# syguan96/DynaBOA

Measured on AMD Instinct MI355X. Metric: adapted frames/sec, whole job (3 inner + 1 outer step, bs=1 per sequence, first-order; synthetic 224x224 stream, no 3DPW assets in the image: PA-MPJPE on 3DPW not measured), higher is better.
Workload: dtype f32

## Files before the change

dynaboa_amd/csrc/adapt_step.hip:

```cpp
#include <math.h>
#include <stdlib.h>
#include <string.h>

#include <algorithm>
#include <chrono>
#include <string>
#include <vector>

#include "dyb_common.h"
#include "dyb_stepper_options.h"

extern "C" {
size_t dyb_hmr_param_floats(const void*);
size_t dyb_hmr_act_floats(const void*);
size_t dyb_hmr_workspace_bytes(const void*);
int dyb_hmr_forward_train(void*, const float*, const float*, const float*, int, float*, void*, size_t, unsigned long long, unsigned long long, float,
                          hipStream_t);
long long dyb_hmr_act_offset_rotmat(const void*);
long long dyb_hmr_act_offset_state(const void*);
size_t dyb_lbs_saved_floats(int);
size_t dyb_lbs_bwd_workspace_bytes(int);
int dyb_lbs_fwd(const float* const*, const int* const*, const float*, int, const float*, float*, float*, float*, int, hipStream_t);
int dyb_lbs_bwd(const float* const*, const int* const*, const float*, const float*, const float*, const float*, float*, float*, int,
                int, void*, size_t, hipStream_t);
// ... 222 lines not shown
  int teacher_train = 0;
  unsigned long long drop_seed = 0, drop_off = 0;
  long long drop_used = 0;
  double drop_p = 0.5;
  volatile float* gate_host = nullptr;
  float* gate_log = nullptr;
  float* feat5_out = nullptr;
  int (*retrieve)(void*, int, const void**) = nullptr;
  int (*retrieve_rep)(void*, int, int, const void**) = nullptr;
  void* retrieve_user = nullptr;
  const float *bank_img = nullptr, *bank_kp = nullptr, *bank_pose = nullptr, *bank_betas = nullptr, *bank_pose3d = nullptr;
  const float *bank_centers = nullptr, *bank_inv_norm = nullptr;
  const int *bank_member_ptr = nullptr, *bank_member_idx = nullptr;
  int* bank_picks = nullptr;
  int bank_items = 0, bank_clusters = 0, bank_members = 0, bank_pick_capacity = 0, bank_on_device = 1;
  unsigned long long bank_seed = 0;
  unsigned long long bank_draw[DYB_MAX_REPLICAS] = {};
  char* retr_ws = nullptr;
  FeatCosArgs fca{};
  float gate_seq = 0.f;
  Pass lvl0{}, ex{}, hist{}, teach{};
  float *grads2 = nullptr, *grads3 = nullptr, *zeros = nullptr, *ex_rot = nullptr;
  const float *lvl_g2 = nullptr, *lvl_g3 = nullptr;
  float *ext_rot = nullptr, *ext_shape = nullptr, *ext_cam = nullptr, *ext_joints = nullptr;
  float *exg_rot = nullptr, *exg_shape = nullptr, *exg_cam = nullptr, *exg_joints = nullptr;
  float *hg_cam = nullptr, *hg_joints = nullptr;
  float *vals_t = nullptr, *vals_m = nullptr, *vals_l = nullptr;
  int nrep = 1;
  int active[DYB_MAX_REPLICAS] = {};
  int nactive = 0;
  long long adam_t_rep[DYB_MAX_REPLICAS] = {};
  size_t blob = 0;
  float* in_stage[12] = {};
  double lr = 3e-6, beta1 = 0.5, beta2 = 0.9, eps = 1e-8, fastlr = 8e-6, w2d = 10.0, wshape = 2e-6, wpose = 1e-4;
  long long adam_t = 0;
  float *theta = nullptr, *adam_m = nullptr, *adam_v = nullptr;
  const float* init_state = nullptr;
  const float* smpl_f[3][7] = {};
  const int* smpl_i[3][3] = {};
  const float *gmm_means = nullptr, *gmm_prec = nullptr, *gmm_logw = nullptr, *j_h36m = nullptr;
  const int* j14 = nullptr;
  float *records = nullptr, *loss_log = nullptr;
  const char* logs_base = nullptr;
  size_t logs_bytes = 0;
  int record_capacity = 0, loss_capacity = 0;
  float* results = nullptr;
  int result_capacity = 0;
  char* wsp = nullptr;
  bool bound = false;
  Pass main{}, fin{};
  float *theta_fast = nullptr, *grads = nullptr;
  float* theta_fast2 = nullptr;
  int fuse_fast = 1;
  std::vector<DybSpan> fused_spans, upd_spans;
  int fuse_adam = 1;
  int fuse_ema = 1;
  float* adam_sc = nullptr;
  bool adam_prepared = false;
  float pre_ss[DYB_MAX_REPLICAS], pre_bc[DYB_MAX_REPLICAS];
  float *gt_rot = nullptr, *gt_verts[3] = {}, *gt_joints = nullptr, *gt_saved = nullptr, *gt17[2] = {};
  DybEvents* ev = nullptr;
  hipEvent_t e_theta = nullptr, e_side = nullptr, e_gt = nullptr;
  int upd_overlap = 1;
  int par_passes = 1, par_max_replicas = DYB_MAX_REPLICAS;
  hipStream_t par_stream[2] = {nullptr, nullptr};
  hipEvent_t par_ev[9] = {nullptr, nullptr, nullptr, nullptr, nullptr, nullptr, nullptr, nullptr, nullptr};
  bool out_in_main = false;
  int share_dyn_fwd = 1;
  hipEvent_t e_upd = nullptr;
  DybFwdGates gates{};
  bool gates_pending = false;
  int wgrad_defer = 1;
  bool defer_pending = false;
  int n_deferred = 0;
  int upd_late = 1;
  struct Upd {
    bool adam = false, ema = false;
    const float *g2 = nullptr, *g3 = nullptr;
    const float* p = nullptr;
    float* out = nullptr;
    float ss[DYB_MAX_REPLICAS] = {}, bc[DYB_MAX_REPLICAS] = {};
  };
  struct LateUpd {
    Upd u;
    hipStream_t aux = nullptr;
    DybRep scope{};
  } late;
  size_t grp_bounds[2] = {0, 0};
  bool side_pending = false;
  struct Tail {
    bool on = false;
    const float* image = nullptr;
    const long long* gender = nullptr;
    int slot = 0;
    bool metrics = false;
    int loss_slot = -1;
  } tail;
  struct GtJob {
    bool on = false;
    const float *pose = nullptr, *betas = nullptr;
  } gtjob;
  hipStream_t tail_stream = nullptr;
  std::string err;
  double h_fwd = 0, h_bwd = 0, h_head = 0, h_update = 0, h_tail = 0, h_total = 0;
  long long h_frames = 0;
};
struct HostTimer {
  double& acc;
  std::chrono::steady_clock::time_point t0;
  explicit HostTimer(double& a) : acc(a), t0(std::chrono::steady_clock::now()) {}
  ~HostTimer() { acc += std::chrono::duration<double, std::milli>(std::chrono::steady_clock::now() - t0).count(); }
};

static size_t a64(size_t v) { return (v + 63) & ~(size_t)63; }
#define BANK_MAX_CHUNKS 256
static bool bank_bound(const Stepper& S) { return S.bank_img && S.bank_on_device; }
static const char* opt_env(const char* name) { return name ? getenv(name) : nullptr; }

static size_t carve(Stepper& S, char* base) {
  size_t off = 0;
  auto take_f = [&](size_t nfloats) -> float* {
    float* p = base ? reinterpret_cast<float*>(base + off) : nullptr;
    off += a64(nfloats) * sizeof(float);
    return p;
  };
  auto take_b = [&](size_t nbytes) -> char* {
    char* p = base ? base + off : nullptr;
    off += a64((nbytes + 3) / 4) * sizeof(float);
    return p;
  };
  const size_t B = (size_t)S.B;
  auto pass = [&](Pass& P, bool with_grad) {
    P.acts = take_f(S.act_floats);
// ... 20 lines not shown
  pass(S.main, true);
  pass(S.fin, false);
  S.theta_fast = take_f(S.n_params);
  S.theta_fast2 = S.fuse_fast ? take_f(S.n_params) : nullptr;
  S.adam_sc = take_f(64);
  S.grads = take_f(S.n_params);
  S.gt_rot = take_f(B * 24 * 9);
  for (int i = 0; i < 3; ++i) S.gt_verts[i] = take_f(B * NV * 3);
  S.gt_joints = take_f(B * NJ * 3);
  S.gt_saved = take_f(S.lbs_saved);
  S.gt17[0] = take_f(B * 51);
  S.gt17[1] = take_f(B * 51);
  if (S.full) {
    S.lvl0 = S.main;
    S.lvl0.acts = take_f(S.act_floats);
    pass(S.ex, true);
    pass(S.hist, true);
    pass(S.teach, false);
    S.grads2 = take_f(S.n_params);
    S.grads3 = take_f(S.n_params);
    S.zeros = take_f(B * 216);
    S.ex_rot = take_f(B * 216);
    S.ext_rot = take_f(B * 216); S.ext_shape = take_f(B * 10); S.ext_cam = take_f(B * 3); S.ext_joints = take_f(B * NJ * 3);
    S.exg_rot = take_f(B * 216); S.exg_shape = take_f(B * 10); S.exg_cam = take_f(B * 3); S.exg_joints = take_f(B * NJ * 3);
    S.hg_cam = take_f(B * 3); S.hg_joints = take_f(B * NJ * 3);
    S.vals_t = take_f(8); S.vals_m = take_f(8); S.vals_l = take_f(8);
  }
  if (S.nrep > 1) {
    S.in_stage[0] = take_f(B * 3 * (size_t)S.H * S.W);
    S.in_stage[1] = take_f(B * NJ * 3);
    S.in_stage[2] = take_f(B * 72);
    S.in_stage[3] = take_f(B * 10);
    S.in_stage[4] = take_f(B * 2);
    if (S.full) {
      S.in_stage[5] = take_f(B * 3 * (size_t)S.H * S.W);
      S.in_stage[6] = take_f(B * NJ * 3);
      S.in_stage[7] = take_f(B * 3 * (size_t)S.H * S.W);
      S.in_stage[8] = take_f(B * NJ * 3);
      S.in_stage[9] = take_f(B * 72);
      S.in_stage[10] = take_f(B * 10);
      S.in_stage[11] = take_f(B * 24 * 4);
    }
  } else if (S.full && S.bank_img) {
    S.in_stage[7] = take_f(B * 3 * (size_t)S.H * S.W);
    S.in_stage[8] = take_f(B * NJ * 3);
    S.in_stage[9] = take_f(B * 72);
    S.in_stage[10] = take_f(B * 10);
    S.in_stage[11] = take_f(B * 24 * 4);
  }
  S.retr_ws = (S.full && S.bank_img) ? take_b(dyb_retrieve_workspace_bytes(S.nrep, BANK_MAX_CHUNKS, 1)) : nullptr;
  return off;
}

extern "C" int dyb_stepper_create(void* plan, int B, int H, int W, void** out) {
  DYB_REQUIRE(plan && out && B > 0 && B <= 64, DYB_ERR_ARG);
  Stepper* S = new Stepper();
  S->plan = plan; S->B = B; S->H = H; S->W = W;
  S->n_params = dyb_hmr_param_floats(plan);
  S->act_floats = dyb_hmr_act_floats(plan);
  S->ws_bytes = dyb_hmr_workspace_bytes(plan);
  S->off_rot = (size_t)dyb_hmr_act_offset_rotmat(plan);
  S->off_state = (size_t)dyb_hmr_act_offset_state(plan);
  S->lbs_saved = dyb_lbs_saved_floats(B);
  S->lbs_wsb = dyb_lbs_bwd_workspace_bytes(B);
  S->ev = dyb_hmr_events_create(plan);
  dyb_hmr_param_groups(plan, S->grp_bounds);
#define DYB_OPT_ENV_(member, name, env, type, locked, doc) \
  if (const char* e = opt_env(env)) S->member = atoi(e);
  DYB_STEPPER_OPTIONS_I(DYB_OPT_ENV_)
#undef DYB_OPT_ENV_
  if (!S->ev || hipEventCreateWithFlags(&S->e_theta, hipEventDisableTiming) != hipSuccess ||
      hipEventCreateWithFlags(&S->e_side, hipEventDisableTiming) != hipSuccess ||
      hipEventCreateWithFlags(&S->e_gt, hipEventDisableTiming) != hipSuccess ||
      hipEventCreateWithFlags(&S->e_upd, hipEventDisableTiming) != hipSuccess ||
      hipEventCreateWithFlags(&S->gates.ev[0], hipEventDisableTiming) != hipSuccess ||
      hipEventCreateWithFlags(&S->gates.ev[1], hipEventDisableTiming) != hipSuccess ||
      hipEventCreateWithFlags(&S->gates.mid, hipEventDisableTiming) != hipSuccess ||
      hipEventCreateWithFlags(&S->ev->l4, hipEventDisableTiming) != hipSuccess ||
      hipEventCreateWithFlags(&S->ev->reg, hipEventDisableTiming) != hipSuccess) {
    delete S;
    return DYB_ERR_LAUNCH;
  }
  *out = S;
  return DYB_OK;
}
extern "C" void dyb_stepper_destroy(void* stepper) {
  Stepper* S = reinterpret_cast<Stepper*>(stepper);
  if (!S) return;
  dyb_hmr_events_destroy(S->ev);
  if (S->e_theta) (void)hipEventDestroy(S->e_theta);
  if (S->e_side) (void)hipEventDestroy(S->e_side);
  if (S->e_gt) (void)hipEventDestroy(S->e_gt);
  if (S->e_upd) (void)hipEventDestroy(S->e_upd);
  if (S->gates.ev[0]) (void)hipEventDestroy(S->gates.ev[0]);
  if (S->gates.ev[1]) (void)hipEventDestroy(S->gates.ev[1]);
  if (S->gates.mid) (void)hipEventDestroy(S->gates.mid);
  for (int i = 0; i < 9; ++i) if (S->par_ev[i]) (void)hipEventDestroy(S->par_ev[i]);
  for (int i = 0; i < 2; ++i) if (S->par_stream[i]) (void)hipStreamDestroy(S->par_stream[i]);
  delete S;
}

extern "C" int dyb_stepper_set_i(void* stepper, const char* key, long long v) {
  Stepper* S = reinterpret_cast<Stepper*>(stepper);
  DYB_REQUIRE(S && key, DYB_ERR_ARG);
  const std::string k(key);
#define DYB_OPT_SET_I_(member, name, env, type, locked, doc) \
  if (k == name) {                                           \
    DYB_REQUIRE(!(locked) || !S->bound, DYB_ERR_ARG);        \
    S->member = (int)v;                                      \
    return DYB_OK;                                           \
  }
  DYB_STEPPER_OPTIONS_I(DYB_OPT_SET_I_)
#undef DYB_OPT_SET_I_
  if (k == "adam_step") {
    S->adam_t = v;
    for (int r = 0; r < DYB_MAX_REPLICAS; ++r) S->adam_t_rep[r] = v;
  }
  else if (k.compare(0, 10, "adam_step_") == 0) {
    const int r = atoi(k.c_str() + 10);
    DYB_REQUIRE(r >= 0 && r < DYB_MAX_REPLICAS, DYB_ERR_ARG);
    S->adam_t_rep[r] = v;
    S->adam_t = 0;
    for (int q = 0; q < S->nrep || q <= r; ++q)
      if (S->adam_t_rep[q] > S->adam_t) S->adam_t = S->adam_t_rep[q];
  }
// ... 195 lines not shown
  for (int g = 0; g < 3; ++g)
    RUN(dyb_lbs_fwd(S.smpl_f[g], S.smpl_i[g], gt_betas, 10, S.gt_rot, S.gt_verts[g], S.gt_joints, S.gt_saved, S.B, st));
  RUN(dyb_regress_joints(S.j_h36m, S.gt_verts[1], S.gt17[0], 17, S.B, st));
  return dyb_regress_joints(S.j_h36m, S.gt_verts[2], S.gt17[1], 17, S.B, st);
}
static int record_metrics(Stepper& S, Pass& P, const long long* gender, int slot, hipStream_t st) {
  DYB_REQUIRE(slot >= 0 && slot < S.record_capacity, DYB_ERR_ARG);
  RUN(dyb_regress_joints(S.j_h36m, P.verts, P.pred17, 17, S.B, st));
  float* rec = S.records + (size_t)slot * a64((size_t)S.B * 85 + 1);
  const DybRep& Rp = dyb_rep_current();
  hipLaunchKernelGGL(metric_record_kernel, dim3(1, 1, Rp.n), dim3(256), 0, st, P.pred17, S.gt17[0], S.gt17[1], gender, S.j14, P.verts,
                     S.gt_verts[0], rec, S.B, Rp);
  DYB_CHECK_LAUNCH();
  return DYB_OK;
}

static int pack_result(Stepper& S, Pass& P, int loss_slot, hipStream_t st) {
  if (!S.results || loss_slot < 0) return DYB_OK;
  float* row = S.results + (size_t)(loss_slot % S.result_capacity) * S.B * RESULT_FLOATS;
  return dyb_result_pack(P.acts + S.off_rot, P.acts + S.off_state, P.verts, row, S.B, st);
}

static int issue_side_work(Stepper& S, hipStream_t side) {
  if (S.tail.on) {
    HIPOK(hipStreamWaitEvent(side, S.e_theta, 0));
    RUN(pass_forward(S, S.fin, S.theta, S.tail.image, side, false));
    if (S.tail.metrics) RUN(record_metrics(S, S.fin, S.tail.gender, S.tail.slot, side));
    RUN(pack_result(S, S.fin, S.tail.loss_slot, side));
    HIPOK(hipEventRecord(S.e_side, side));
    S.side_pending = true;
    S.tail.on = false;
  }
  if (S.gtjob.on) {
    RUN(gt_meshes(S, S.gtjob.pose, S.gtjob.betas, side));
    HIPOK(hipEventRecord(S.e_gt, side));
    S.gtjob.on = false;
  }
  return DYB_OK;
}
static bool spans_touch(const Stepper& S, size_t lo, size_t hi) {
  for (const DybSpan& sp : S.upd_spans)
    if (sp.off < hi && sp.off + sp.n > lo) return true;
  return false;
}
template <class Emit>
static int walk_gaps(const Stepper& S, size_t lo, size_t hi, Emit emit) {
  DYB_REQUIRE(lo % 4 == 0 && hi % 4 == 0, DYB_ERR_UNSUPPORTED);
  DybFwSegs t{};
  auto flush = [&]() -> int {
    if (t.n == 0) return DYB_OK;
    const int rc = emit(t);
    t.n = 0;
    return rc;
  };
  auto add = [&](size_t a, size_t b) -> int {
    if (a >= b) return DYB_OK;
    DYB_REQUIRE(a % 4 == 0 && b % 4 == 0 && (b - a) / 4 < 0xffffffffull && a / 4 < 0xffffffffull, DYB_ERR_UNSUPPORTED);
    if (t.n == DYB_FW_MAX_SEGS) RUN(flush());
    t.start4[t.n] = (unsigned)(a / 4); t.count4[t.n] = (unsigned)((b - a) / 4); ++t.n;
    return DYB_OK;
  };
  size_t at = lo;
  for (const DybSpan& sp : S.upd_spans) {
    if (sp.off + sp.n <= at) continue;
    if (sp.off >= hi) break;
    DYB_REQUIRE(sp.off >= lo && sp.off + sp.n <= hi, DYB_ERR_UNSUPPORTED);
// ... 300 lines not shown
        const void* one[5] = {nullptr, nullptr, nullptr, nullptr, nullptr};
        if (S.retrieve_rep(S.retrieve_user, level_index, r, one) != 0) return DYB_ERR_ARG;
        for (int k = 0; k < 5; ++k) {
          DYB_REQUIRE(one[k], DYB_ERR_ARG);
          exin[k * DYB_MAX_REPLICAS + r] = one[k];
        }
      }
      RUN(stage_inputs(S, exin, DYB_MAX_REPLICAS, IN_EX_IMG, 5, st));
      for (int k = 0; k < 5; ++k) C.in[IN_EX_IMG + k] = S.in_stage[IN_EX_IMG + k];
    } else if (S.retrieve) {
      DYB_REQUIRE(S.feat5_out && S.nrep == 1, DYB_ERR_ARG);
      RUN(dyb_scale_add(nullptr, P.acts + S.fca.off[5], nullptr, S.feat5_out, (size_t)0 + (size_t)B * 2048, st));
      const void* exin[5] = {nullptr, nullptr, nullptr, nullptr, nullptr};
      if (S.retrieve(S.retrieve_user, level_index, exin) != 0) return DYB_ERR_ARG;
      for (int k = 0; k < 5; ++k) C.in[IN_EX_IMG + k] = exin[k];
    }
    DYB_REQUIRE(C.in[IN_EX_IMG] && C.in[IN_EX_KP] && C.in[IN_EX_POSE] && C.in[IN_EX_BETAS] && C.in[IN_EX_POSE3D], DYB_ERR_ARG);
    RUN(label_pass_forward_and_term(st, true));
  }
  if (C.losslog && S.full) {
    if (par && label) HIPOK(hipStreamWaitEvent(st, S.par_ev[4], 0));
    hipLaunchKernelGGL(level_log_kernel, dim3(1, 1, dyb_rep_current().n), dim3(64), 0, st, (const float*)P.losses,
                       teacher ? (const float*)S.vals_t : nullptr, motion ? (const float*)S.vals_m : nullptr,
                       label ? (const float*)S.vals_l : nullptr, (float)S.teacher_w, (float)S.motion_w, (float)S.label_w,
                       C.losslog + 16 * level_index, dyb_rep_current());
    DYB_CHECK_LAUNCH();
  }
  {
    HostTimer t(S.h_bwd);
    S.fused_spans.clear();
    DybWgradUpdate upd{};
    if (fused_epilogues(S) && !upper && S.fuse_fast && S.theta_fast2) {
      upd = DybWgradUpdate{S.grads, S.n_params * sizeof(float), cur, nxt, (float)S.fastlr, &S.fused_spans};
    } else if (fused_epilogues(S) && upper && S.fuse_adam && cur != S.theta && !C.side && S.nrep > 1) {
      RUN(adam_prepare(S, st));
      upd = DybWgradUpdate{S.grads, S.n_params * sizeof(float), S.theta, S.theta, 0.f, &S.fused_spans};
      upd.adam_m = S.adam_m; upd.adam_v = S.adam_v; upd.adam_sc = S.adam_sc;
      upd.b1 = (float)S.beta1; upd.b2 = (float)S.beta2; upd.eps = (float)S.eps;
    }
    DybWgradUpdateScope fuse(upd);
    RUN(pass_backward_ext(S, P, cur, S.grads, true, ext ? S.ext_rot : nullptr, ext ? S.ext_shape : nullptr, ext ? S.ext_cam : nullptr,
                          ext ? S.ext_joints : nullptr, st, aux));
  }
  S.lvl_g2 = S.lvl_g3 = nullptr;
  if (motion) {
    if (par) HIPOK(hipStreamWaitEvent(st, S.par_ev[3], 0));
    else RUN(pass_backward_ext(S, S.hist, cur, S.grads2, false, nullptr, nullptr, S.hg_cam, S.hg_joints, st, aux));
    S.lvl_g2 = S.grads2;
  }
  if (label) {
    if (par) HIPOK(hipStreamWaitEvent(st, S.par_ev[5], 0));
    else RUN(pass_backward_ext(S, S.ex, cur, S.grads3, false, S.exg_rot, S.exg_shape, S.exg_cam, S.exg_joints, st, aux));
    if (S.lvl_g2) S.lvl_g3 = S.grads3;
    else S.lvl_g2 = S.grads3;
  }
  tails.armed = false;
  return DYB_OK;
}
static int outer_update(Stepper& S, hipStream_t st, hipStream_t aux) {
  return weight_update(S, true, nullptr, nullptr, st, aux, S.full && S.use_teacher && S.teacher);
}
static int gate_cosine(Stepper& S, const float* actsA, const float* actsB, float* log_row, float* cos12, hipStream_t st) {
  DYB_REQUIRE(S.gate_host, DYB_ERR_ARG);
  const DybRep& R = dyb_rep_current();
  S.gate_seq += 1.f;
  hipLaunchKernelGGL(feat_cos_kernel, dim3(15, 1, R.n), dim3(1024), 0, st, actsA, actsB, S.fca, 1e-12f, log_row, S.gate_host, S.gate_seq, R);
  DYB_CHECK_LAUNCH();
// ... 54 lines not shown
    arena(S.loss_log, (size_t)S.loss_capacity * (S.full ? 16 : 4) * rows * sizeof(float));
    if (S.full) {
      arena(S.gate_log, (size_t)S.loss_capacity * (1 + S.optim_steps) * 16 * sizeof(float));
      arena(S.feat5_out, (size_t)S.B * 2048 * sizeof(float));
    }
  }
  DYB_REQUIRE(!overflow, DYB_ERR_UNSUPPORTED);
  *out = R;
  return DYB_OK;
}
extern "C" int dyb_stepper_set_active(void* stepper, const int* idx, int n) {
  Stepper* S = reinterpret_cast<Stepper*>(stepper);
  DYB_REQUIRE(S && n >= 0 && n <= S->nrep && (n == 0 || idx), DYB_ERR_ARG);
  for (int i = 0; i < n; ++i) DYB_REQUIRE(idx[i] >= 0 && idx[i] < S->nrep && (i == 0 || idx[i] > idx[i - 1]), DYB_ERR_ARG);
  S->nactive = n;
  for (int i = 0; i < n; ++i) S->active[i] = idx[i];
  return DYB_OK;
}
static int active_set(const Stepper& S, int* idx) {
  if (S.nactive > 0) {
    for (int i = 0; i < S.nactive; ++i) idx[i] = S.active[i];
    return S.nactive;
  }
  for (int i = 0; i < S.nrep; ++i) idx[i] = i;
  return S.nrep;
}

static int frame_step(Stepper& S, LevelCtx& C, int record_slot, int loss_slot, int* extra, hipStream_t st, hipStream_t aux, hipStream_t side) {
  const bool metrics = S.metrics != 0;
  DYB_REQUIRE(C.in[IN_IMAGE] && C.in[IN_KP], DYB_ERR_ARG);
  DYB_REQUIRE(!metrics || (C.in[IN_GT_POSE] && C.in[IN_GT_BETAS] && C.in[IN_GENDER]), DYB_ERR_ARG);
  S.out_in_main = false;
  if (!S.use_side || side == st) side = nullptr;
  const float* image = (const float*)C.in[IN_IMAGE];
  const long long* gender = (const long long*)C.in[IN_GENDER];
  const int K = S.inner_step;
  const int rows = K + 1 + (S.full && S.dynamic ? S.optim_steps : 0);
  C.losslog = (S.loss_log && loss_slot >= 0 && loss_slot < S.loss_capacity) ? S.loss_log + (size_t)loss_slot * (S.full ? 16 : 4) * rows : nullptr;
  C.side = side;
  int slot = record_slot;
  const DybRep outer = dyb_rep_current();
  for (int i = 0; i < outer.n; ++i) extra[dyb_rep_phys(outer, i)] = 0;
  if (metrics) {
    if (side) {
      S.gtjob.on = true; S.gtjob.pose = (const float*)C.in[IN_GT_POSE]; S.gtjob.betas = (const float*)C.in[IN_GT_BETAS];
    } else {
      RUN(gt_meshes(S, (const float*)C.in[IN_GT_POSE], (const float*)C.in[IN_GT_BETAS], st));
    }
  }
  C.gt_waited = !(metrics && side);
  HostTimer t_all(S.h_total);
  ++S.h_frames;
  const float* cur = S.theta;
  for (int i = 0; i <= K; ++i) {
    Pass& P = (i == 0 && S.full && S.dynamic) ? S.lvl0 : S.main;
    float* nxt = (fused_epilogues(S) && S.fuse_fast && S.theta_fast2 && cur == S.theta_fast) ? S.theta_fast2 : S.theta_fast;
    RUN(level(S, C, P, cur, nxt, i == K, i, (metrics && S.eval_lower && i > 0) ? slot++ : -1, st, aux));
    if (i == 0 && side) {
      HostTimer t(S.h_tail);
      RUN(issue_side_work(S, side));
    }
    if (i < K) {
      HostTimer t(S.h_update);
      RUN(weight_update(S, false, cur, nxt, st, aux));
      cur = nxt;
    }
  }
  {
    HostTimer t_tail(S.h_tail);
    if (S.side_pending) {
      HIPOK(hipStreamWaitEvent(st, S.e_side, 0));
      S.side_pending = false;
    }
    RUN(outer_update(S, st, side ? nullptr : aux));
    if (side) {
      HIPOK(hipEventRecord(S.e_theta, st));
      S.tail.on = true; S.tail.image = image; S.tail.gender = gender; S.tail.slot = slot++; S.tail.metrics = metrics;
      S.tail.loss_slot = loss_slot;
      S.tail_stream = side;
      return DYB_OK;
    }
    RUN(pass_forward(S, S.fin, S.theta, image, st));
    RUN(settle_update(S, st));
    if (metrics) RUN(record_metrics(S, S.fin, gender, slot++, st));
    RUN(pack_result(S, S.fin, loss_slot, st));
  }
  if (!(S.full && S.dynamic)) return DYB_OK;
  float* glog = (S.gate_log && loss_slot >= 0 && loss_slot < S.loss_capacity) ? S.gate_log + (size_t)loss_slot * (1 + S.optim_steps) * 16 : nullptr;
  DYB_REQUIRE(glog, DYB_ERR_ARG);
  float cos12[DYB_MAX_REPLICAS];
  RUN(gate_cosine(S, S.lvl0.acts, S.fin.acts, glog, cos12, st));
  int cont[DYB_MAX_REPLICAS], ncont = 0;
  for (int i = 0; i < outer.n; ++i)
    if (1.f - cos12[dyb_rep_phys(outer, i)] > (float)S.cos_thr) cont[ncont++] = dyb_rep_phys(outer, i);
  int step = 0;
  Pass* post = &S.fin;
  while (ncont > 0) {
    ++step;
    if (step > S.optim_steps) {
      for (int i = 0; i < ncont; ++i) extra[cont[i]] = S.optim_steps + 1;
      break;
    }
    {
      DybRep sub = outer;
      dyb_rep_set_map(sub, cont, ncont);
      DybRepScope scope(sub);
      Pass up = S.main;
// ... 10 lines not shown
      RUN(pack_result(S, *nxt, loss_slot, st));
      post = nxt;
      S.out_in_main = (post == &S.main);
    }
    ++slot;
    int m = 0;
    for (int i = 0; i < ncont; ++i) {
      extra[cont[i]] = step;
      if (1.f - cos12[cont[i]] > (float)S.cos_thr) cont[m++] = cont[i];
    }
    ncont = m;
  }
  return DYB_OK;
}
static int adapt(Stepper& S, const void* const* inputs, int nk, int record_slot, int loss_slot, int* extra_steps, hipStream_t st,
                 hipStream_t aux, hipStream_t side) {
  RUN(check_ready(S));
  DYB_REQUIRE((nk == IN_COUNT) == (S.full != 0) && (!S.full || S.B <= 16), DYB_ERR_UNSUPPORTED);
  struct DrawGuard {
    Stepper& S;
    unsigned long long saved[DYB_MAX_REPLICAS];
    bool ok = false;
    explicit DrawGuard(Stepper& s) : S(s) { memcpy(saved, S.bank_draw, sizeof saved); }
    ~DrawGuard() { if (!ok) memcpy(S.bank_draw, saved, sizeof saved); }
  } draws(S);
  const int n = S.nrep;
  int extra[DYB_MAX_REPLICAS] = {};
  LevelCtx C{};
  int rc;
  if (n == 1) {
    for (int k = 0; k < nk; ++k) C.in[k] = inputs[k];
    rc = frame_step(S, C, record_slot, loss_slot, extra, st, aux, side);
  } else {
    DYB_REQUIRE(!(S.use_side && side && side != st), DYB_ERR_UNSUPPORTED);
    int act[DYB_MAX_REPLICAS];
    const int na = active_set(S, act);
    auto have = [&](int r, int k0, int k1) {
      for (int k = k0; k <= k1; ++k)
        if (k >= nk || !inputs[k * n + r]) return false;
      return true;
    };
    const bool have_gt = have(act[0], IN_GT_POSE, IN_GENDER), have_hist = have(act[0], IN_HIST_IMAGE, IN_HIST_KP),
               have_ex = have(act[0], IN_EX_IMG, IN_EX_POSE3D);
    for (int i = 0; i < na; ++i) {
      DYB_REQUIRE(have(act[i], IN_IMAGE, IN_KP), DYB_ERR_ARG);
      DYB_REQUIRE(have(act[i], IN_GT_POSE, IN_GENDER) == have_gt && have(act[i], IN_HIST_IMAGE, IN_HIST_KP) == have_hist &&
                  have(act[i], IN_EX_IMG, IN_EX_POSE3D) == have_ex, DYB_ERR_UNSUPPORTED);
    }
    DybRep R{};
    RUN(make_scope(S, act, na, &R));
    DybRepScope scope(R);
    RUN(stage_inputs(S, inputs, n, IN_IMAGE, 5, st));
    if (have_hist) RUN(stage_inputs(S, inputs + (size_t)IN_HIST_IMAGE * n, n, IN_HIST_IMAGE, 2, st));
    if (have_ex) RUN(stage_inputs(S, inputs + (size_t)IN_EX_IMG * n, n, IN_EX_IMG, 5, st));
    for (int k = 0; k < nk; ++k) {
      const bool on = k <= IN_KP || (k <= IN_GENDER ? have_gt : k <= IN_HIST_KP ? have_hist : have_ex);
      C.in[k] = on ? S.in_stage[k] : nullptr;
    }
    rc = frame_step(S, C, record_slot, loss_slot, extra, st, aux, side);
  }
  if (extra_steps)
    for (int r = 0; r < n; ++r) extra_steps[r] = extra[r];
  draws.ok = rc == DYB_OK;
  return rc;
}
extern "C" int dyb_stepper_adapt_frame(void* stepper, const float* image, const float* kp2d, const float* gt_pose,
                                       const float* gt_betas, const long long* gender, int record_slot, int loss_slot,
                                       hipStream_t st, hipStream_t aux, hipStream_t side) {
  Stepper* S = reinterpret_cast<Stepper*>(stepper);
  DYB_REQUIRE(S && image && kp2d && S->nrep == 1, DYB_ERR_ARG);
  const void* inputs[5] = {image, kp2d, gt_pose, gt_betas, gender};
  return adapt(*S, inputs, 5, record_slot, loss_slot, nullptr, st, aux, side);
}
extern "C" int dyb_stepper_adapt_frames(void* stepper, const void* const* inputs, int record_slot, int loss_slot, hipStream_t st,
                                        hipStream_t aux, hipStream_t side) {
  Stepper* S = reinterpret_cast<Stepper*>(stepper);
  DYB_REQUIRE(S && inputs, DYB_ERR_ARG);
  return adapt(*S, inputs, 5, record_slot, loss_slot, nullptr, st, aux, side);
}
extern "C" int dyb_stepper_adapt_frame_full(void* stepper, const void* const* inputs, int record_slot, int loss_slot, int* extra_steps,
                                            hipStream_t st, hipStream_t aux) {
  Stepper* S = reinterpret_cast<Stepper*>(stepper);
  DYB_REQUIRE(S && inputs && extra_steps, DYB_ERR_ARG);
  DYB_REQUIRE(S->nrep == 1, DYB_ERR_UNSUPPORTED);
  return adapt(*S, inputs, IN_COUNT, record_slot, loss_slot, extra_steps, st, aux, nullptr);
// ... 31 lines not shown
```

dynaboa_amd/csrc/dyb_stepper_options.h:

```cpp
#pragma once
#define DYB_STEPPER_OPTIONS_I(X)                                                                                                              \
  X(n_iter, "n_iter", nullptr, I, 0, "iterations of the HMR regressor (1 .. 3)")                                                              \
  X(inner_step, "inner_step", nullptr, I, 0, "lower levels per frame (0 .. 16)")                                                              \
  X(eval_lower, "eval_lower", nullptr, I, 0, "a metric record after every inner step")                                                        \
  X(use_side, "use_side", nullptr, I, 0, "one sequence, frame-loss set: final inference and ground-truth meshes on the side stream")          \
  X(metrics, "metrics", nullptr, I, 0, "metric records at all")                                                                               \
  X(upd_overlap, "upd_overlap", "DYB_UPD_OVERLAP", I, 0, "replica groups: weight updates by arena ranges beside the next forward")            \
  X(upd_late, "upd_late", "DYB_UPD_LATE", I, 0, "the last range (layer4 + regressor) is issued when the consuming forward reaches layer3")    \
  X(wgrad_defer, "wgrad_defer", "DYB_WGRAD_DEFER", I, 0, "layer4 / regressor weight gradients behind the backward's join, beside the next forward") \
  X(fuse_fast, "fuse_fast", "DYB_FUSE_FAST", I, 1, "frame-loss set: lower levels' weight gradients write the fast weights themselves (second fast buffer)") \
  X(fuse_adam, "fuse_adam", "DYB_FUSE_ADAM", I, 0, "frame-loss set, replica groups: the outer level's weight gradients apply Adam in place")  \
  X(fuse_ema, "fuse_ema", "DYB_FUSE_EMA", I, 0, "the teacher's EMA inside the Adam pass")                                                     \
  X(par_passes, "par_passes", "DYB_PAR_PASSES", I, 0, "full set: history and exemplar passes on two streams of the stepper's own")            \
  X(par_max_replicas, "par_max_replicas", "DYB_PAR_MAX_REPLICAS", I, 0, "largest launch set that still runs the parallel passes")             \
  X(share_dyn_fwd, "share_dyn_fwd", "DYB_SHARE_DYN_FWD", I, 0, "dynamic loop: a step's upper level reuses the previous final inference as its forward") \
  X(full, "full", nullptr, I, 1, "the reference's full term set (teacher / motion / labelled exemplars / dynamic loop): sizes the workspace")  \
  X(temporal_lower, "temporal_lower", nullptr, I, 0, "teacher / motion terms on the lower levels")                                            \
  X(temporal_upper, "temporal_upper", nullptr, I, 0, "teacher / motion terms on the upper level")                                             \
  X(use_teacher, "use_teacher", nullptr, I, 0, "mean-teacher term and the teacher's EMA")                                                     \
  X(teacher_train, "teacher_train", nullptr, I, 0, "teacher forwards with live dropout (keys: drop_seed, drop_offset)")                       \
  X(use_motion, "use_motion", nullptr, I, 0, "motion term against the frame `interval` steps back")                                           \
  X(interval, "interval", nullptr, I, 0, "distance of the history frame (bookkeeping of the caller)")                                         \
  X(mix_lower, "mix_lower", nullptr, I, 0, "labelled-exemplar term on the lower levels")                                                      \
  X(mix_upper, "mix_upper", nullptr, I, 0, "labelled-exemplar term on the upper level")                                                       \
  X(dynamic, "dynamic", nullptr, I, 0, "dynamic loop: repeat the upper level while feature 12 still moves")                                   \
  X(optim_steps, "optim_steps", nullptr, I, 0, "its iteration limit")                                                                         \
  X(kp_set, "kp_set", nullptr, I, 0, "keypoint window of the 2D term and the motion term: 0 gt24 (joints 25..48) | 1 op25 (joints 0..24)")   \
  X(record_capacity, "record_capacity", nullptr, I, 0, "metric-record slots behind `records`")                                                \
  X(loss_capacity, "loss_capacity", nullptr, I, 0, "frames behind `loss_log` / `gate_log`")                                                   \
  X(result_capacity, "result_capacity", nullptr, I, 0, "rows behind `results` (a frame's final inferences go to row loss_slot mod this)")      \
  X(bank_items, "bank_items", nullptr, I, 0, "exemplar bank: items in the five tables")                                                       \
  X(bank_clusters, "bank_clusters", nullptr, I, 0, "exemplar bank: cluster centres")                                                          \
  X(bank_members, "bank_members", nullptr, I, 0, "exemplar bank: entries of bank_member_idx")                                                 \
  X(bank_pick_capacity, "bank_pick_capacity", nullptr, I, 0, "exemplar bank: rows of each replica's pick log (row = draw index mod this)")    \
  X(bank_on_device, "bank_on_device", "DYB_BANK_ON_DEVICE", I, 0, "exemplar bank: 1 select / gather kernels inside the level | 0 ignore the bank (callback route; A/B)")
#define DYB_STEPPER_OPTIONS_F(X)                                                                                                              \
  X(lr, "lr", nullptr, F, 0, "Adam learning rate")                                                                                            \
  X(beta1, "beta1", nullptr, F, 0, "Adam beta1")                                                                                              \
  X(beta2, "beta2", nullptr, F, 0, "Adam beta2")                                                                                              \
  X(eps, "eps", nullptr, F, 0, "Adam epsilon")                                                                                                \
  X(fastlr, "fastlr", nullptr, F, 0, "fast-weight learning rate")                                                                             \
  X(w2d, "s2dloss_weight", nullptr, F, 0, "frame head: 2D keypoint term")                                                                     \
// ... 40 lines not shown
```

dynaboa_amd/native_step.py:

```python
from __future__ import annotations

import os

import ctypes
from typing import Dict, Optional

import torch

from . import _lib
from ._abi import check
from .hmr import get_layout, stream_of
from .losses import kp_set_id


def coverage(o, have_bundle: bool = True):
    g = lambda k, d=0: getattr(o, k, d)
    if not g("use_boa", 1):
        return "", "use_boa=0"
    if g("second_order"):
        return "", "second order"
    if not (g("use_frame_losses_lower", 1) and g("use_frame_losses_upper", 1)):
        return "", "frame losses switched off"
    if g("dump_predictions") and not g("native_results"):
        return "", "prediction dumps"
    if g("save_res") and not g("native_results"):
        return "", "rendered results"
    if not g("share_forwards", 1) or not g("fused_level", 1):
        return "", "unshared / unfused schedule requested"
    temporal = (g("use_temporal_losses_lower") or g("use_temporal_losses_upper")) and (g("use_meanteacher") or g("use_motion"))
    mix = g("lower_level_mixtrain") or g("upper_level_mixtrain")
    if not (temporal or mix or g("dynamic_boa") or g("use_meanteacher")):
        return "frame", None
    B = int(g("batch_size", 1))
    if B > 16:
        return "", "full term set natively needs batch <= 16"
    if mix and not g("retrieval"):
        return "", "labelled term without retrieval"
# ... 32 lines not shown
        L = get_layout(B)
        h = ctypes.c_void_p()
        check(lib.dyb_stepper_create(L.plan, B, 224, 224, ctypes.byref(h)), "dyb_stepper_create")
        self.h = h
        self._keep = []
        si = lambda k, v: check(lib.dyb_stepper_set_i(h, k.encode(), int(v)), f"set_i {k}")
        sf = lambda k, v: check(lib.dyb_stepper_set_f(h, k.encode(), float(v)), f"set_f {k}")

        def sp(k, t):
            self._keep.append(t)
            check(lib.dyb_stepper_set_p(h, k.encode(), t.data_ptr()), f"set_p {k}")
        si("replicas", S)
        self.mode = mode(o, getattr(adaptor, "bundle", None) is not None)
        self.full = self.mode == "full"
        si("inner_step", self.K); si("eval_lower", self.eval_lower); si("n_iter", 3)
        si("kp_set", kp_set_id(getattr(o, "kp_set", "gt24")))
        self.metrics = int(getattr(o, "metrics", 1))
        si("metrics", self.metrics)
        if self.full:
            g = lambda k, d=0: getattr(o, k, d)
            si("full", 1)
            si("temporal_lower", g("use_temporal_losses_lower")); si("temporal_upper", g("use_temporal_losses_upper", 1))
            si("use_teacher", g("use_meanteacher", 1)); si("use_motion", g("use_motion", 1)); si("interval", g("interval", 5))
            si("mix_lower", g("lower_level_mixtrain", 1)); si("mix_upper", g("upper_level_mixtrain", 1))
            si("dynamic", g("dynamic_boa", 1)); si("optim_steps", g("optim_steps", 7))
            for k in ("teacherloss_weight", "motionloss_weight", "labelloss_weight", "alpha", "cos_sim_threshold"):
                sf(k, getattr(o, k))
            self.dynamic, self.optim_steps = int(g("dynamic_boa", 1)), int(g("optim_steps", 7))
            self.teacher_train = bool(g("teacher_dropout")) and bool(g("use_meanteacher", 1))
            if self.teacher_train:
                si("teacher_train", 1)
                sf("drop_p", float(getattr(adaptor.teacher, "dropout_p", 0.5)))
        self.use_side = 1 if (S == 1 and getattr(adaptor, "_side", None) is not None) else 0
        si("use_side", self.use_side)
        for k in ("lr", "beta1", "beta2", "fastlr", "s2dloss_weight", "shape_prior_weight", "pose_prior_weight"):
            sf(k, getattr(o, k))
        sf("eps", adaptor.optimizer.param_groups[0]["eps"])
        n = hmr.theta.numel()
        steps = []
        for a in ads:
            st = a.optimizer.state.get(a.model.module.theta)
            steps.append(0 if st is None else int(st["step"]))
        if S == 1:
            theta = hmr.theta
            st = adaptor.optimizer.state.get(theta)
            if st is None:
                st = adaptor.optimizer.state[theta] = dict(step=0, exp_avg=torch.zeros_like(theta), exp_avg_sq=torch.zeros_like(theta))
            self.theta, self.m, self.v = theta.data, st["exp_avg"], st["exp_avg_sq"]
            self._adam = [st]
        else:
            self.theta = torch.empty(S, n, device=dev)
            self.m, self.v = torch.zeros(S, n, device=dev), torch.zeros(S, n, device=dev)
            self._adam = []
            for r, a in enumerate(ads):
                p = a.model.module.theta
                self.theta[r].copy_(p.data)
                old = a.optimizer.state.get(p)
                if old is not None:
                    self.m[r].copy_(old["exp_avg"]); self.v[r].copy_(old["exp_avg_sq"])
                p.data = self.theta[r]
                a.optimizer.state[p] = dict(step=steps[r], exp_avg=self.m[r], exp_avg_sq=self.v[r])
                self._adam.append(a.optimizer.state[p])
        si("adam_step", steps[0])
        for r, t in enumerate(steps):
            si(f"adam_step_{r}", t)
        sp("theta", self.theta); sp("adam_m", self.m); sp("adam_v", self.v)
# ... 86 lines not shown
                        out[i] = t.data_ptr()
                if S == 1:
                    CB = ctypes.CFUNCTYPE(ctypes.c_int, ctypes.c_void_p, ctypes.c_int, ctypes.POINTER(ctypes.c_void_p))

                    def _retrieve(_user, _level, out):
                        try:
                            _retrieve_one(0, out)
                            return 0
                        except Exception as e:
                            self._cb_error = e
                            return 1
                    key = b"retrieve_fn"
                else:
                    CB = ctypes.CFUNCTYPE(ctypes.c_int, ctypes.c_void_p, ctypes.c_int, ctypes.c_int, ctypes.POINTER(ctypes.c_void_p))

                    def _retrieve(_user, _level, r, out):
                        try:
                            _retrieve_one(int(r), out)
                            return 0
                        except Exception as e:
                            self._cb_error = e
                            return 1
                    key = b"retrieve_rep_fn"
                self._cb = CB(_retrieve)
                check(lib.dyb_stepper_set_p(h, key, ctypes.cast(self._cb, ctypes.c_void_p)), "set_p " + key.decode())
        nbytes = int(lib.dyb_stepper_workspace_bytes(h))
        self.ws = torch.empty(nbytes, dtype=torch.uint8, device=dev)
        check(lib.dyb_stepper_bind_workspace(h, self.ws.data_ptr(), nbytes, stream_of(self.theta)), "dyb_stepper_bind_workspace")
        self.frame = 0
        self._aux = torch.cuda.Stream(device=dev) if dev.type == "cuda" else None
        if os.environ.get("DYB_NO_AUX") == "1":
            self._aux = None

    def __del__(self):
        try:
            if getattr(self, "h", None):
                self.lib.dyb_stepper_destroy(self.h)
                self.h = None
        except Exception:
            pass

    def output(self, which: int, replica: int = 0) -> torch.Tensor:
        self.lib.dyb_stepper_output.restype = ctypes.c_void_p
        p = self.lib.dyb_stepper_output(self.h, int(which))
        if not p:
            raise RuntimeError("dyb_stepper_output: stepper not bound")
        shape = {0: (self.B, 24, 9), 1: (self.B, 160), 2: (self.B, 6890, 3), 3: (self.B, 49, 3)}[int(which)]
        off = int(p) - self.ws.data_ptr() + replica * (self.ws.numel() // self.S)
        n = 1
        for d in shape:
            n *= d
        if off < 0 or off % 4 or off + 4 * n > self.ws.numel():
            raise RuntimeError("dyb_stepper_output: pointer outside the workspace")
        return self.ws[off:off + 4 * n].view(torch.float32).view(shape)

    def result(self, frame: int, replica: int = 0) -> Dict[str, torch.Tensor]:
        if self.results is None:
            raise RuntimeError("native stepper: no result ring (native_results with save_res / dump_predictions)")
        row = self.results[replica, frame % self.result_capacity]
        return dict(vts=row[:, :20670].unflatten(1, (6890, 3)), rotmat=row[:, 20670:20886].unflatten(1, (24, 3, 3)),
                    shape=row[:, 20886:20896], cam=row[:, 20896:20899])

    def _step(self, rows, full: bool, side=None):
        f, S, nk = self.frame, self.S, 12 if full else 5
        if f >= self.loss_log.shape[1]:
            raise RuntimeError("native stepper: more frames than reset_records() announced")
        ptrs = (ctypes.c_void_p * (nk * S))()
        for r, row in rows.items():
            for k, t in enumerate(row):
                ptrs[k * S + r] = None if t is None else t.data_ptr()
        extra = (ctypes.c_int * S)()
        slot0 = f * self.slots_per_frame
        st, aux = stream_of(self.theta), self._aux.cuda_stream if self._aux is not None else None
        if full:
            self._cb_error = None
            self._drop_begin()
            self._bank_begin(rows)
            rc = self.lib.dyb_stepper_adapt_frames_full(self.h, ctypes.cast(ptrs, ctypes.c_void_p), slot0, f, ctypes.cast(extra, ctypes.c_void_p),
                                                        st, aux)
            if getattr(self, "_cb_error", None) is not None:
                raise self._cb_error
            self._drop_end()
            if rc == 0:
                self._bank_end(rows)
        else:
            rc = self.lib.dyb_stepper_adapt_frames(self.h, ctypes.cast(ptrs, ctypes.c_void_p), slot0, f, st, aux, side)
        check(rc, "dyb_stepper_adapt_frames_full" if full else "dyb_stepper_adapt_frames")
        self._sync_adam_steps()
        self._prev_keep, self._keep_inputs = getattr(self, "_keep_inputs", None), rows
        self.frame += 1
        return f, slot0, [int(x) for x in extra]

    def adapt_frames(self, batches, side_stream=None):
        if len(batches) != self.S:
            raise ValueError(f"{self.S} replicas, {len(batches)} batches")
        rows = {r: [b["image"].contiguous().float(), b["smpl_j2d"].contiguous().float()] + self._gt_row(b) for r, b in enumerate(batches)}
        side = None
        if side_stream is not None and self.use_side:
            side = side_stream.cuda_stream
            for row in rows.values():
                for t in row:
                    if t is not None and t.is_cuda:
                        t.record_stream(side_stream)
        return self._step(rows, False, side)[:2]

    def adapt_frame(self, batch: Dict[str, torch.Tensor], side_stream=None):
        return self.adapt_frames([batch], side_stream)

    def _gt_row(self, batch):
        if not self.metrics:
            return [None, None, None]
        return [batch["pose"].contiguous().float(), batch["betas"].contiguous().float(), batch["gender"].contiguous().long()]

    def _full_row(self, batch, hist, exemplars):
        c = lambda t: t if (t.dtype is torch.float32 and t.is_contiguous()) else t.contiguous().float()
        row = [c(batch["image"]), c(batch["smpl_j2d"])] + self._gt_row(batch)
        row += [c(hist[0]), c(hist[1])] if hist is not None else [None, None]
        row += [c(exemplars[k]) for k in ("img", "keypoints", "pose", "betas", "pose_3d")] if exemplars is not None else [None] * 5
        return row

    def adapt_frame_full(self, batch, hist=None, exemplars=None):
        f, slot0, extra = self._step({0: self._full_row(batch, hist, exemplars)}, True)
        return f, slot0, extra[0]

    def _drop_begin(self):
        if getattr(self, "teacher_train", False):
            from . import hmr as _H
            seed = int(torch.initial_seed()) & ((1 << 64) - 1)
            check(self.lib.dyb_stepper_set_i(self.h, b"drop_seed", seed - (1 << 64) if seed >= (1 << 63) else seed), "set_i drop_seed")
            check(self.lib.dyb_stepper_set_i(self.h, b"drop_offset", _H._DROP_CALLS[0] + 1), "set_i drop_offset")

# ... 50 lines not shown
            cos = [[row.unbind(0) for row in rep.unbind(0)] for rep in g.unbind(0)]
            c = self._gate_cache = (frame, cos, [m.unbind(0) for m in means])
        return c[1][r], c[2][r]

    def join(self):
        check(self.lib.dyb_stepper_join(self.h, stream_of(self.theta)), "dyb_stepper_join")

    def _frame_record_views(self, slot: int):
        T, B, S = self.slots_per_frame, self.B, self.S
        f = slot // T
        c = getattr(self, "_rec_cache", None)
        if c is None or c[0] != f:
            R = self.records[:, f * T:(f + 1) * T]
            cols = (R[..., :B * 42].view(S, T, B, 14, 3), R[..., B * 42:B * 84].view(S, T, B, 14, 3), R[..., B * 84:B * 85], R[..., B * 85])
            per = [[t.unbind(0) for t in col.unbind(0)] for col in cols]
            c = self._rec_cache = (f, per)
        return c[1]

    def record_views(self, slot: int, r: int = 0):
        per = self._frame_record_views(slot)
        k = slot % self.slots_per_frame
        return dict(pred=per[0][r][k], gt=per[1][r][k], mpjpe=per[2][r][k], pve=per[3][r][k])

    def losses(self, frame: int, level: int, r: int = 0):
        if self.full:
            return self.loss_log[r, frame, 4 * level:4 * level + 4]
        c = getattr(self, "_loss_cache", None)
        if c is None or c[0] != frame:
            rows = self.loss_log[:, frame].view(self.S, -1, 4)
            c = self._loss_cache = (frame, [t.unbind(0) for t in rows.unbind(0)])
        return c[1][r][level]


RESULT_RING_ROWS = 2
BANK_PICK_ROWS = 256


TP_MIN_SEQUENCES = int(os.environ.get("DYB_TP_MIN_SEQUENCES", "5"))


def set_replica_policy(throughput: bool = True):
    lib = _lib.load()
    check(lib.dyb_set_option(b"rep_split", 1 if throughput else 0), "dyb_set_option rep_split")
    if throughput:
        check(lib.dyb_set_option(b"tp_min", TP_MIN_SEQUENCES), "dyb_set_option tp_min")


class ReplicaGroup:

    def __init__(self, adaptors, nframes: int):
        why = supported(adaptors[0].options)
        if why:
            raise ValueError(f"replica groups need a configuration the native stepper covers ({why})")
        for a in adaptors:
            a.reset_records(nframes)
            a._native_why = ""
        self.adaptors = list(adaptors)
        self.stepper = NativeStepper(self.adaptors, nframes)
        for r, a in enumerate(self.adaptors):
            a._native, a._native_replica = self.stepper, r

    def step(self, batches, global_step: int, result_steps=None):
        ns = self.stepper
        active = [r for r, b in enumerate(batches) if b is not None]
        if not active:
            return [None] * len(batches)
        if len(active) != len(batches) or getattr(ns, "active", None) not in (None, active):
            ns.set_active(active)
        for r in active:
            a, b = self.adaptors[r], batches[r]
            a.global_step = global_step
            a._result_step = None if result_steps is None else int(result_steps[r])
            a.fit_losses = {}
            a.save_hist(b["image"], b["smpl_j2d"])
        out = [None] * len(batches)
        if ns.full:
            ins = {r: self.adaptors[r]._native_full_inputs(batches[r]) for r in active}
            hists = [ins[r][0] if r in ins else None for r in range(len(batches))]
            exs = [ins[r][1] if r in ins else None for r in range(len(batches))]
            f, slot, extra = ns.adapt_frames_full(batches, hists, exs)
            for r in active:
                out[r] = self.adaptors[r]._native_full_bookkeeping(f, slot, extra[r], hists[r])
        else:
            full = [b if b is not None else batches[active[0]] for b in batches]
            f, slot = ns.adapt_frames(full)
            for r in active:
                out[r] = self.adaptors[r]._native_bookkeeping(f, slot)
        if ns.results is not None:
            self._write_results(f, active, batches)
        return out

    def _write_results(self, f, active, batches):
        from .base_adaptor import draw_overlays
        jobs = []
        for r in active:
            a, b = self.adaptors[r], batches[r]
            res = self.stepper.result(f, r)
            if getattr(a.options, "dump_predictions", 0):
                a.dump_prediction(res["vts"], res["cam"], res["rotmat"], res["shape"])
            if getattr(a.options, "save_res", 0):
                jobs += a.overlay_jobs(res["vts"], res["cam"], b["image"], b.get("imgname"), b.get("bbox"), prefix="Pred")
        if jobs:
            draw_overlays(self.adaptors[active[0]].ragged_renderer(), jobs, self.adaptors[active[0]].RESULT_COLOR)

    def flush_metrics(self):
        from .benchmark import flush_metrics_of
        return flush_metrics_of(self.adaptors)
```

Before: 502.0.

## Run replica-group final inference on a side stream beside the next frame

For replica groups in the frame-loss configuration, the final inference, settle, metrics and result packing after the outer update now run on a dedicated side stream. This lets them overlap with the next frame's first inner level. Double-buffered input staging buffers are added so the next frame's staging does not overwrite inputs the side stream still reads. Events order Adam, ground-truth meshes and the side work, and the Python side creates one side stream per process-wide group. The change adds synchronisation complexity and memory, and allows only one active group to use the feature at a time.

```diff
diff --git a/dynaboa_amd/csrc/adapt_step.hip b/dynaboa_amd/csrc/adapt_step.hip
--- a/dynaboa_amd/csrc/adapt_step.hip
+++ b/dynaboa_amd/csrc/adapt_step.hip
@@ -278,6 +278,7 @@
   long long adam_t_rep[DYB_MAX_REPLICAS] = {};
   size_t blob = 0;
   float* in_stage[12] = {};
+  float* in_stage_alt[5] = {};
   double lr = 3e-6, beta1 = 0.5, beta2 = 0.9, eps = 1e-8, fastlr = 8e-6, w2d = 10.0, wshape = 2e-6, wpose = 1e-4;
   long long adam_t = 0;
   float *theta = nullptr, *adam_m = nullptr, *adam_v = nullptr;
@@ -307,6 +308,7 @@
   float *gt_rot = nullptr, *gt_verts[3] = {}, *gt_joints = nullptr, *gt_saved = nullptr, *gt17[2] = {};
   DybEvents* ev = nullptr;
   hipEvent_t e_theta = nullptr, e_side = nullptr, e_gt = nullptr;
+  hipEvent_t e_stage = nullptr;
   int upd_overlap = 1;
   int par_passes = 1, par_max_replicas = DYB_MAX_REPLICAS;
   hipStream_t par_stream[2] = {nullptr, nullptr};
@@ -320,6 +322,7 @@
   bool defer_pending = false;
   int n_deferred = 0;
   int upd_late = 1;
+  int group_side = 1;
   struct Upd {
     bool adam = false, ema = false;
     const float *g2 = nullptr, *g3 = nullptr;
@@ -345,6 +348,7 @@
   struct GtJob {
     bool on = false;
     const float *pose = nullptr, *betas = nullptr;
+    bool staged = false;
   } gtjob;
   hipStream_t tail_stream = nullptr;
   std::string err;
@@ -431,6 +435,13 @@
     S.in_stage[2] = take_f(B * 72);
     S.in_stage[3] = take_f(B * 10);
     S.in_stage[4] = take_f(B * 2);
+    if (!S.full) {
+      S.in_stage_alt[0] = take_f(B * 3 * (size_t)S.H * S.W);
+      S.in_stage_alt[1] = take_f(B * NJ * 3);
+      S.in_stage_alt[2] = take_f(B * 72);
+      S.in_stage_alt[3] = take_f(B * 10);
+      S.in_stage_alt[4] = take_f(B * 2);
+    }
     if (S.full) {
       S.in_stage[5] = take_f(B * 3 * (size_t)S.H * S.W);
       S.in_stage[6] = take_f(B * NJ * 3);
@@ -471,6 +482,7 @@
   if (!S->ev || hipEventCreateWithFlags(&S->e_theta, hipEventDisableTiming) != hipSuccess ||
       hipEventCreateWithFlags(&S->e_side, hipEventDisableTiming) != hipSuccess ||
       hipEventCreateWithFlags(&S->e_gt, hipEventDisableTiming) != hipSuccess ||
+      hipEventCreateWithFlags(&S->e_stage, hipEventDisableTiming) != hipSuccess ||
       hipEventCreateWithFlags(&S->e_upd, hipEventDisableTiming) != hipSuccess ||
       hipEventCreateWithFlags(&S->gates.ev[0], hipEventDisableTiming) != hipSuccess ||
       hipEventCreateWithFlags(&S->gates.ev[1], hipEventDisableTiming) != hipSuccess ||
@@ -490,6 +502,7 @@
   if (S->e_theta) (void)hipEventDestroy(S->e_theta);
   if (S->e_side) (void)hipEventDestroy(S->e_side);
   if (S->e_gt) (void)hipEventDestroy(S->e_gt);
+  if (S->e_stage) (void)hipEventDestroy(S->e_stage);
   if (S->e_upd) (void)hipEventDestroy(S->e_upd);
   if (S->gates.ev[0]) (void)hipEventDestroy(S->gates.ev[0]);
   if (S->gates.ev[1]) (void)hipEventDestroy(S->gates.ev[1]);
@@ -751,6 +764,7 @@
     S.tail.on = false;
   }
   if (S.gtjob.on) {
+    if (S.gtjob.staged) HIPOK(hipStreamWaitEvent(side, S.e_stage, 0));
     RUN(gt_meshes(S, S.gtjob.pose, S.gtjob.betas, side));
     HIPOK(hipEventRecord(S.e_gt, side));
     S.gtjob.on = false;
@@ -1117,7 +1131,11 @@
     DybWgradUpdate upd{};
     if (fused_epilogues(S) && !upper && S.fuse_fast && S.theta_fast2) {
       upd = DybWgradUpdate{S.grads, S.n_params * sizeof(float), cur, nxt, (float)S.fastlr, &S.fused_spans};
-    } else if (fused_epilogues(S) && upper && S.fuse_adam && cur != S.theta && !C.side && S.nrep > 1) {
+    } else if (fused_epilogues(S) && upper && S.fuse_adam && cur != S.theta && S.nrep > 1) {
+      if (S.side_pending) {
+        HIPOK(hipStreamWaitEvent(st, S.e_side, 0));
+        S.side_pending = false;
+      }
       RUN(adam_prepare(S, st));
       upd = DybWgradUpdate{S.grads, S.n_params * sizeof(float), S.theta, S.theta, 0.f, &S.fused_spans};
       upd.adam_m = S.adam_m; upd.adam_v = S.adam_v; upd.adam_sc = S.adam_sc;
@@ -1238,6 +1256,7 @@
   DYB_REQUIRE(!metrics || (C.in[IN_GT_POSE] && C.in[IN_GT_BETAS] && C.in[IN_GENDER]), DYB_ERR_ARG);
   S.out_in_main = false;
   if (!S.use_side || side == st) side = nullptr;
+  if (!side && (S.tail.on || S.gtjob.on) && S.tail_stream && S.tail_stream != st) RUN(issue_side_work(S, S.tail_stream));
   const float* image = (const float*)C.in[IN_IMAGE];
   const long long* gender = (const long long*)C.in[IN_GENDER];
   const int K = S.inner_step;
@@ -1250,7 +1269,12 @@
   if (metrics) {
     if (side) {
       S.gtjob.on = true; S.gtjob.pose = (const float*)C.in[IN_GT_POSE]; S.gtjob.betas = (const float*)C.in[IN_GT_BETAS];
+      S.gtjob.staged = S.nrep > 1;
     } else {
+      if (S.side_pending) {
+        HIPOK(hipStreamWaitEvent(st, S.e_side, 0));
+        S.side_pending = false;
+      }
       RUN(gt_meshes(S, (const float*)C.in[IN_GT_POSE], (const float*)C.in[IN_GT_BETAS], st));
     }
   }
@@ -1278,7 +1302,29 @@
       HIPOK(hipStreamWaitEvent(st, S.e_side, 0));
       S.side_pending = false;
     }
-    RUN(outer_update(S, st, side ? nullptr : aux));
+    RUN(outer_update(S, st, (side && S.nrep == 1) ? nullptr : aux));
+    if (side && S.nrep > 1) {
+      hipEvent_t done[4] = {nullptr, nullptr, nullptr, nullptr};
+      if (S.gates_pending) {
+        if (S.gates.late) {
+          HIPOK(hipEventRecord(S.gates.mid, st));
+          RUN(late_update(&S));
+        }
+        done[0] = S.gates.ev[0]; done[1] = S.gates.ev[1]; done[2] = S.gates.l4; done[3] = S.gates.reg;
+      }
+      HIPOK(hipEventRecord(S.e_theta, st));
+      for (hipEvent_t e : done)
+        if (e) HIPOK(hipStreamWaitEvent(st, e, 0));
+      HIPOK(hipStreamWaitEvent(side, S.e_theta, 0));
+      RUN(pass_forward(S, S.fin, S.theta, image, side));
+      RUN(settle_update(S, side));
+      if (metrics) RUN(record_metrics(S, S.fin, gender, slot++, side));
+      RUN(pack_result(S, S.fin, loss_slot, side));
+      HIPOK(hipEventRecord(S.e_side, side));
+      S.side_pending = true;
+      S.tail_stream = side;
+      return DYB_OK;
+    }
     if (side) {
       HIPOK(hipEventRecord(S.e_theta, st));
       S.tail.on = true; S.tail.image = image; S.tail.gender = gender; S.tail.slot = slot++; S.tail.metrics = metrics;
@@ -1355,7 +1401,10 @@
     for (int k = 0; k < nk; ++k) C.in[k] = inputs[k];
     rc = frame_step(S, C, record_slot, loss_slot, extra, st, aux, side);
   } else {
-    DYB_REQUIRE(!(S.use_side && side && side != st), DYB_ERR_UNSUPPORTED);
+    DYB_REQUIRE(!(S.use_side && side && side != st && S.full), DYB_ERR_UNSUPPORTED);
+    if (!S.group_side) side = nullptr;
+    if (S.in_stage_alt[0])
+      for (int k = 0; k < 5; ++k) std::swap(S.in_stage[k], S.in_stage_alt[k]);
     int act[DYB_MAX_REPLICAS];
     const int na = active_set(S, act);
     auto have = [&](int r, int k0, int k1) {
@@ -1374,6 +1423,7 @@
     RUN(make_scope(S, act, na, &R));
     DybRepScope scope(R);
     RUN(stage_inputs(S, inputs, n, IN_IMAGE, 5, st));
+    if (side && side != st) HIPOK(hipEventRecord(S.e_stage, st));
     if (have_hist) RUN(stage_inputs(S, inputs + (size_t)IN_HIST_IMAGE * n, n, IN_HIST_IMAGE, 2, st));
     if (have_ex) RUN(stage_inputs(S, inputs + (size_t)IN_EX_IMG * n, n, IN_EX_IMG, 5, st));
     for (int k = 0; k < nk; ++k) {
diff --git a/dynaboa_amd/csrc/dyb_stepper_options.h b/dynaboa_amd/csrc/dyb_stepper_options.h
--- a/dynaboa_amd/csrc/dyb_stepper_options.h
+++ b/dynaboa_amd/csrc/dyb_stepper_options.h
@@ -3,11 +3,12 @@
   X(n_iter, "n_iter", nullptr, I, 0, "iterations of the HMR regressor (1 .. 3)")                                                              \
   X(inner_step, "inner_step", nullptr, I, 0, "lower levels per frame (0 .. 16)")                                                              \
   X(eval_lower, "eval_lower", nullptr, I, 0, "a metric record after every inner step")                                                        \
-  X(use_side, "use_side", nullptr, I, 0, "one sequence, frame-loss set: final inference and ground-truth meshes on the side stream")          \
+  X(use_side, "use_side", nullptr, I, 0, "frame-loss set: final inference and ground-truth meshes on the side stream (groups: with group_side)") \
   X(metrics, "metrics", nullptr, I, 0, "metric records at all")                                                                               \
   X(upd_overlap, "upd_overlap", "DYB_UPD_OVERLAP", I, 0, "replica groups: weight updates by arena ranges beside the next forward")            \
   X(upd_late, "upd_late", "DYB_UPD_LATE", I, 0, "the last range (layer4 + regressor) is issued when the consuming forward reaches layer3")    \
   X(wgrad_defer, "wgrad_defer", "DYB_WGRAD_DEFER", I, 0, "layer4 / regressor weight gradients behind the backward's join, beside the next forward") \
+  X(group_side, "group_side", "DYB_GROUP_SIDE", I, 0, "replica groups, frame-loss set: the final inference on the side stream, beside the next frame's first level") \
   X(fuse_fast, "fuse_fast", "DYB_FUSE_FAST", I, 1, "frame-loss set: lower levels' weight gradients write the fast weights themselves (second fast buffer)") \
   X(fuse_adam, "fuse_adam", "DYB_FUSE_ADAM", I, 0, "frame-loss set, replica groups: the outer level's weight gradients apply Adam in place")  \
   X(fuse_ema, "fuse_ema", "DYB_FUSE_EMA", I, 0, "the teacher's EMA inside the Adam pass")                                                     \
diff --git a/dynaboa_amd/native_step.py b/dynaboa_amd/native_step.py
--- a/dynaboa_amd/native_step.py
+++ b/dynaboa_amd/native_step.py
@@ -3,6 +3,7 @@
 import os
 
 import ctypes
+import weakref
 from typing import Dict, Optional
 
 import torch
@@ -101,6 +102,24 @@
                 si("teacher_train", 1)
                 sf("drop_p", float(getattr(adaptor.teacher, "dropout_p", 0.5)))
         self.use_side = 1 if (S == 1 and getattr(adaptor, "_side", None) is not None) else 0
+        self._side = None
+        gs = getattr(o, "group_side", None)
+        if gs is not None:
+            si("group_side", int(gs))
+        self.group_side = int(lib.dyb_stepper_get_i(h, b"group_side"))
+        if S > 1 and self.group_side and not self.full:
+            import gc
+            if len(_SIDE_GROUPS):
+                gc.collect()
+            for other in list(_SIDE_GROUPS):
+                other._group_side_off()
+            if len(_SIDE_GROUPS):
+                self.group_side = 0
+                si("group_side", 0)
+            _SIDE_GROUPS.add(self)
+        if S > 1 and self.group_side and not self.full:
+            self._side = torch.cuda.Stream(device=dev) if dev.type == "cuda" else None
+            self.use_side = 1
         si("use_side", self.use_side)
         for k in ("lr", "beta1", "beta2", "fastlr", "s2dloss_weight", "shape_prior_weight", "pose_prior_weight"):
             sf(k, getattr(o, k))
@@ -253,6 +272,11 @@
         if os.environ.get("DYB_NO_AUX") == "1":
             self._aux = None
 
+    def _group_side_off(self):
+        if self.group_side and getattr(self, "h", None):
+            check(self.lib.dyb_stepper_set_i(self.h, b"group_side", 0), "set_i group_side")
+            self.group_side = 0
+
     def __del__(self):
         try:
             if getattr(self, "h", None):
@@ -317,7 +341,10 @@
             raise ValueError(f"{self.S} replicas, {len(batches)} batches")
         rows = {r: [b["image"].contiguous().float(), b["smpl_j2d"].contiguous().float()] + self._gt_row(b) for r, b in enumerate(batches)}
         side = None
-        if side_stream is not None and self.use_side:
+        if self.S > 1:
+            if self.use_side and self._side is not None:
+                side = self._side.cuda_stream
+        elif side_stream is not None and self.use_side:
             side = side_stream.cuda_stream
             for row in rows.values():
                 for t in row:
@@ -434,6 +461,7 @@
         return c[1][r][level]
 
 
+_SIDE_GROUPS = weakref.WeakSet()
 RESULT_RING_ROWS = 2
 BANK_PICK_ROWS = 256
 
@@ -494,6 +522,7 @@
 
     def _write_results(self, f, active, batches):
         from .base_adaptor import draw_overlays
+        self.stepper.join()
         jobs = []
         for r in active:
             a, b = self.adaptors[r], batches[r]
```

Result: faster. 508.0 (median of 6 runs) (+1.2%).
